# zaiisao/ConTEXTure-NeRF

Measured on AMD Instinct MI355X. Metric: UNet denoise steps/sec (CFG-batched SD2-depth UNet eval + PLMS update), higher is better.
Workload: dtype f16; 1 GPU; BASELINE configs[1]: 1 view @768^2 (latent 96^2), 50 PLMS steps (51 UNet evals), SD2-depth UNet fp16, CFG batch 2, guidance 10, random-init weights; mesh substitution napoleon.obj -> n/a for this stage (denoise loop only); latent=96, cfg_batch=2, ctx_len=77, views_per_rank=1, parallelism=view-shard x1

## Files before the change

contexture-nerf_amd/_lib.py:

```python
import ctypes as C
import os
import torch

_HERE = os.path.dirname(os.path.abspath(__file__))
LIB_PATH = os.path.join(_HERE, "libctxnerf.so")

_vp, _i32, _i64, _f32 = C.c_void_p, C.c_int32, C.c_int64, C.c_float

SIGNATURES = {
    "ctx_version": (_i32, []),
    "ctx_last_error": (C.c_char_p, []),
    "ctx_device_check": (_i32, []),
    "ctx_prepare_vertices": (_i32, [_vp, _vp, _vp, _vp, _i32, _i32, _i32, _vp, _vp, _vp, _vp, _vp]),
    "ctx_rasterize_ws_bytes": (_i64, [_i32, _i32, _i32, _i32]),
    "ctx_rasterize_fwd": (_i32, [_i32, _i32, _vp, _vp, _vp, _i32, _i32, _i32, _f32, _f32, _vp, _vp, _vp, _i64, _vp]),
    "ctx_rasterize_fused": (_i32, [_i32, _i32, _vp, _vp, _vp, _i32, _vp, _i32, _i32, _f32, _f32, _vp, _vp, _vp, _vp, _vp, _i64, _vp]),
    "ctx_normalize_depth_ws_bytes": (_i64, [_i32]),
    "ctx_normalize_depth": (_i32, [_vp, _i32, _i32, _vp, _vp, _vp, _vp]),
    "ctx_texture_mapping_fwd": (_i32, [_vp, _vp, _i32, _i32, _i32, _i32, _i32, _i32, _vp, _vp, _vp]),
    "ctx_texture_mapping_bwd": (_i32, [_vp, _vp, _i32, _i32, _i32, _i32, _vp, _vp, _vp]),
    "ctx_texmap_bwd_plan_bytes": (_i64, [_i32, _i32, _i32]),
    "ctx_texmap_bwd_plan": (_i32, [_vp, _vp, _i32, _i32, _i32, _vp, _vp]),
    "ctx_texture_mapping_bwd_binned_ws_bytes": (_i64, [_i32, _i32]),
    "ctx_texture_mapping_bwd_binned": (_i32, [_vp, _vp, _vp, _i32, _i32, _i32, _i32, _vp, _vp, _vp, _vp]),
# ... 86 lines not shown
    "ctx_unet_set_param": (_i32, [_vp, _i32, _vp, _vp]),
    "ctx_unet_forward": (_i32, [_vp, _vp, _vp, _vp, _i32, _i32, _i32, _i32, _vp, _vp]),
    "ctx_controlnet_create": (_vp, [_vp, _i32]),
    "ctx_controlnet_residual_bytes": (_i64, [_vp, _i32, _i32, _i32]),
    "ctx_controlnet_cond_cache_bytes": (_i64, [_vp, _i32, _i32, _i32]),
    "ctx_controlnet_forward": (_i32, [_vp, _vp, _vp, _vp, _vp, _vp, _i32, _i32, _i32, _i32, _i32, _vp, _vp]),
    "ctx_unet_set_residuals": (_i32, [_vp, _vp, C.c_float]),
    "ctx_unet_ref_bank_bytes": (_i64, [_vp, _i32, _i32, _i32]),
    "ctx_unet_workspace_bytes_ref": (_i64, [_vp, _i32, _i32, _i32, _i32, _i32, _i32]),
    "ctx_unet_forward_ref": (_i32, [_vp, _vp, _vp, _vp, _i32, _i32, _i32, _i32, _i32, _vp, _i32, _vp, _vp]),
    "ctx_unet_set_residual_fp32": (_i32, [_vp, _i32]),
    "ctx_unet_stats": (_i32, [_vp, _i32, _vp, _vp]),
    "ctx_unet_gn_epilogue_counts": (_i32, [_vp, _vp, _vp]),
    "ctx_unet_set_taps": (_i32, [_vp, _vp, _i64]),
    "ctx_unet_tap_count": (_i32, [_vp]),
    "ctx_unet_tap_info": (_i32, [_vp, _i32, _vp, _vp, _vp]),
    "ctx_vae_create": (_vp, [_vp]),
    "ctx_vae_destroy": (None, [_vp]),
    "ctx_vae_param_count": (_i32, [_vp]),
    "ctx_vae_param_name": (C.c_char_p, [_vp, _i32]),
    "ctx_vae_param_shape": (_i32, [_vp, _i32, _vp]),
    "ctx_vae_weight_bytes": (_i64, [_vp]),
    "ctx_vae_workspace_bytes": (_i64, [_vp, _i32, _i32, _i32]),
    "ctx_vae_bind": (_i32, [_vp, _vp, _vp, _i64]),
    "ctx_vae_derived_bytes": (_i64, [_vp]),
    "ctx_vae_bind_derived": (_i32, [_vp, _vp, _i64]),
    "ctx_vae_set_param": (_i32, [_vp, _i32, _vp, _vp]),
    "ctx_vae_decode": (_i32, [_vp, _vp, _i32, _i32, _i32, _vp, _vp]),
    "ctx_vae_decoder_param_count": (_i32, [_vp]),
    "ctx_vae_encode_workspace_bytes": (_i64, [_vp, _i32, _i32, _i32]),
    "ctx_vae_encode": (_i32, [_vp, _vp, _i32, _i32, _i32, _vp, _vp]),
    "ctx_vae_flops": (C.c_double, [_vp]),
    "ctx_vae_encode_train_workspace_bytes": (_i64, [_vp, _i32, _i32, _i32]),
    "ctx_vae_encode_train": (_i32, [_vp, _vp, _i32, _i32, _i32, _vp, _vp]),
    "ctx_vae_encode_bwd": (_i32, [_vp, _vp, _f32, _vp, _vp]),
    "ctx_gemm_f16": (_i32, [_vp, _vp, _vp, _vp, _i32, _i32, _i32, _vp, _vp]),
    "ctx_conv3x3_f16": (_i32, [_vp, _vp, _vp, _vp, _vp, _i32, _i32, _i32, _i32, _i32, _i32, _i32, _vp, _vp]),
    "ctx_conv3x3_seg_f16": (_i32, [_vp, _vp, _vp, _vp, _vp, _vp, _i32, _i32, _i32, _i32, _i32, _vp, _vp, _i32, _i32, _vp, _vp, _i32, _i32,
                                   _vp, _i32, _vp, _vp]),
    "ctx_conv3x3_gn_f16": (_i32, [_vp, _vp, _vp, _vp, _vp, _vp, _i32, _i32, _i32, _i32, _i32, _vp, _i32, _i32, _i32, _vp, _vp, _vp, _vp]),
    "ctx_gemm_last_kernel": (None, [_vp, _vp]),
    "ctx_conv3x3_geom_f16": (_i32, [_vp, _vp, _vp, _vp, _i32, _i32, _i32, _i32, _i32, _i32, _i32, _i32, _i32, _vp, _i32, _vp, _vp]),
    "ctx_pack_conv3_dgrad_f16": (_i32, [_vp, _i32, _i32, _i32, _vp, _vp]),
    "ctx_pack_conv3_phase_f16": (_i32, [_vp, _i32, _i32, _vp, _vp]),
    "ctx_conv3x3_phase_f16": (_i32, [_vp, _vp, _vp, _vp, _vp, _i32, _i32, _i32, _i32, _i32, _vp, _i32, _vp, _vp]),
    "ctx_pack_mat_dgrad_f16": (_i32, [_vp, _i32, _i32, _i32, _i32, _vp, _vp]),
    "ctx_groupnorm_bwd_ws_bytes": (_i64, [_i32, _i32]),
    "ctx_groupnorm_bwd_f16": (_i32, [_vp, _vp, _vp, _vp, _vp, _i32, _i32, _i32, _i32, _f32, _i32, _vp, _vp, _vp]),
    "ctx_softmax_rows_f16": (_i32, [_vp, _i32, _i32, _f32, _vp, _vp]),
    "ctx_softmax_bwd_rows_f16": (_i32, [_vp, _vp, _i32, _i32, _f32, _vp, _vp]),
    "ctx_quant_bwd_f16": (_i32, [_vp, _vp, _i32, _i32, _i64, _f32, _vp, _vp]),
    "ctx_conv_in_bwd_f16": (_i32, [_vp, _vp, _i32, _i32, _i32, _i32, _i32, _f32, _vp, _vp]),
    "ctx_conv_in_f16": (_i32, [_vp, _vp, _vp, _i32, _i32, _i32, _i32, _i32, _vp, _vp]),
    "ctx_conv_out_f16": (_i32, [_vp, _vp, _vp, _i32, _i32, _i32, _i32, _i32, _vp, _vp]),
    "ctx_gemv_f16": (_i32, [_vp, _vp, _vp, _i32, _i32, _i32, _i32, _i32, _vp, _vp]),
    "ctx_time_embed_f16": (_i32, [_vp, _i32, _i32, _vp, _vp]),
    "ctx_transpose_v_f16": (_i32, [_vp, _i32, _i32, _i32, _i32, _i32, _vp, _vp]),
    "ctx_concat_f16": (_i32, [_vp, _vp, _i64, _i32, _i32, _vp, _vp]),
    "ctx_concat_f32": (_i32, [_vp, _vp, _i64, _i32, _i32, _vp, _vp]),
    "ctx_f32_to_f16": (_i32, [_vp, _i64, _vp, _vp]),
    "ctx_f16_to_f32": (_i32, [_vp, _i64, _vp, _vp]),
    "ctx_conv_small_f16": (_i32, [_vp, _vp, _vp, _vp, _i32, _i32, _i32, _i32, _i32, _i32, _i32, _vp, _vp]),
    "ctx_add_scaled_f16": (_i32, [_vp, _vp, _f32, _i64, _vp]),
    "ctx_pointwise_f32": (_i32, [_vp, _vp, _vp, _i32, _i32, _i64, _i32, _vp, _vp]),
    "ctx_pack_fwd_f16": (_i32, [_vp, _i32, _i32, _i32, _vp, _vp]),
    "ctx_groupnorm_f16": (_i32, [_vp, _vp, _vp, _i32, _i32, _i32, _i32, _f32, _i32, _vp, _vp, _vp]),
    "ctx_groupnorm2_f16": (_i32, [_vp, _vp, _i32, _vp, _vp, _i32, _i32, _i32, _i32, _f32, _i32, _vp, _vp, _vp]),
    "ctx_groupnorm_apply_f16": (_i32, [_vp, _vp, _i32, _vp, _vp, _i32, _i32, _i32, _i32, _f32, _i32, _vp, _vp]),
    "ctx_groupnorm_slabs_f16": (_i32, [_vp, _i32, _vp, _vp, _vp, _i32, _vp, _vp, _i32, _i32, _i32, _i32, _f32, _i32, _vp, _vp]),
    "ctx_layernorm_f16": (_i32, [_vp, _vp, _vp, _i64, _i32, _f32, _vp, _vp]),
    "ctx_groupnorm_plan": (_i32, [_i32, _i32, _i32, _i32, _i32, _i32, _vp]),
    "ctx_layernorm_plan": (_i32, [_i64, _i32, _i32, _vp]),
    "ctx_groupnorm_f32in_f16": (_i32, [_vp, _vp, _vp, _i32, _i32, _i32, _i32, _f32, _i32, _vp, _vp, _vp]),
    "ctx_layernorm_f32in_f16": (_i32, [_vp, _vp, _vp, _i64, _i32, _f32, _vp, _vp]),
    "ctx_attention_ws_bytes": (_i64, [_i32, _i32, _i32]),
    "ctx_attention_f16": (_i32, [_vp, _vp, _vp, _i32, _i32, _i32, _i32, _i32, _i32, _f32, _vp, _i32, _vp, _vp]),
    "ctx_groupnorm_ws_bytes": (_i64, [_i32, _i32]),
    "ctx_geglu_f16": (_i32, [_vp, _i64, _i32, _vp, _vp]),
    "ctx_profile_begin": (_i32, []),
    "ctx_profile_end": (_i32, [_i32, _vp, _vp]),
    "ctx_bench_gemm": (C.c_float, [_vp, _vp, _vp, _vp, _i32, _i32, _i32, _vp, _i32, _i32, _i32, _i32, _i32, _i32, _vp, _i32, _i32, _vp]),
    "ctx_gemm_tune": (None, [_i32, _i32]),
    "ctx_attention_tune": (None, [_i32, _i32, _i32, _f32]),
    "ctx_probe_mfma": (_i32, [_i32, _vp, _vp, _vp, _vp]),
    "ctx_probe_stage": (C.c_float, [_i32, _i32, _i32, _i32, _i32, _vp, _vp, _vp]),
    "ctx_cfg_plms_step": (_i32, [_vp, _i64, _f32, _vp, _i32, _vp, _f32, _f32, _i32, _vp, _vp, _vp]),
}


class CtxError(RuntimeError):
    pass


_lib = None


def load():
    global _lib
    if _lib is None:
        if not os.path.exists(LIB_PATH):
            raise CtxError(f"{LIB_PATH} is missing: run `python -c 'import __graft_entry__ as g; g.build()'` "
                           "(hipcc --offload-arch=gfx950). There is no CPU fallback for this path.")
        lib = C.CDLL(LIB_PATH)
        for name, (res, args) in SIGNATURES.items():
            if not hasattr(lib, name) and os.environ.get("CTX_ALLOW_PARTIAL") == "1":
                continue
            fn = getattr(lib, name)
            fn.restype = res
            fn.argtypes = args
        _lib = lib
    return _lib


def check(rc):
    if rc != 0:
        raise CtxError(f"libctxnerf error {rc}: {load().ctx_last_error().decode()}")


def stream():
    return C.c_void_p(torch.cuda.current_stream().cuda_stream)


def ptr(t, dtype=None, name="tensor"):
    if t is None:
        return C.c_void_p(0)
    if not isinstance(t, torch.Tensor) or not t.is_cuda:
        raise CtxError(f"{name}: expected a device tensor (the HIP path has no CPU fallback), got "
                       f"{type(t).__name__} on {getattr(t, 'device', '?')}")
    if not t.is_contiguous():
        raise CtxError(f"{name}: tensor must be contiguous")
    if dtype is not None and t.dtype != dtype:
        raise CtxError(f"{name}: expected dtype {dtype}, got {t.dtype}")
    return C.c_void_p(t.data_ptr())


def f32c(t, device=None):
    t = t.to(dtype=torch.float32)
    if device is not None:
        t = t.to(device)
    return t.contiguous()
```

contexture-nerf_amd/csrc/attention.hip:

```cpp
#include "gemm_common.h"
#include <math.h>

#define AT_KB 64
#define AT_KROW 72
#define AT_VROW 68


struct AttnArgs {
    const f16 *Q, *K, *V;
    f16 *O;
    int Sq, Skv, heads;
    int q_stride, kv_stride, o_stride;
    float scale_log2e;
    float lazy;
};



typedef short at_s16x4 __attribute__((__vector_size__(4 * sizeof(short))));
__device__ __forceinline__ f16x4 at_tr16(const f16 *p)
{
    at_s16x4 v = __builtin_amdgcn_ds_read_tr16_b64_v4i16((__attribute__((address_space(3))) at_s16x4 *)p);
    return __builtin_bit_cast(f16x4, v);
}
struct AtNoIssue { __device__ __forceinline__ void operator()(int) const {} };
template <bool MASK, int NISSUE = 0, class Issue = AtNoIssue>
__device__ __forceinline__ void attn_tile(const f16 *__restrict__ Ks, const f16 *__restrict__ Vs, int k0, int Skv, int r, int h,
                                          int swz, int vlane, int vfq, float c, const f16x8 (&qf)[4], f32x16 (&o)[2], f32x16 &ls,
                                          float &m_run, float lazy, Issue iss = Issue())
{
    f32x16 s[2];
#pragma unroll
    for (int kb = 0; kb < 2; ++kb) {
#pragma unroll
        for (int q = 0; q < 16; ++q) s[kb][q] = 0.f;
        const f16 *kr = Ks + (kb * 32 + r) * 64;
#pragma unroll
        for (int ks = 0; ks < 4; ++ks) {
            f16x8 kf = *(const f16x8 *)(kr + ((2 * ks + h) ^ swz) * 8);
            s[kb] = __builtin_amdgcn_mfma_f32_32x32x16_f16(kf, qf[ks], s[kb], 0, 0, 0);
            if (kb * 4 + ks < NISSUE) iss(kb * 4 + ks);
        }
    }
    if (MASK) {
#pragma unroll
        for (int kb = 0; kb < 2; ++kb)
#pragma unroll
            for (int q = 0; q < 16; ++q) {
                int key = k0 + kb * 32 + (q & 3) + 8 * (q >> 2) + 4 * h;
                if (key >= Skv) s[kb][q] = -INFINITY;
            }
    }
    float mxa = fmaxf(s[0][0], s[0][1]), mxb = fmaxf(s[1][0], s[1][1]);
#pragma unroll
    for (int q = 2; q < 16; q += 2) {
        mxa = __builtin_fmaxf(__builtin_fmaxf(mxa, s[0][q]), s[0][q + 1]);
        mxb = __builtin_fmaxf(__builtin_fmaxf(mxb, s[1][q]), s[1][q + 1]);
    }
    float mx = fmaxf(mxa, mxb);
    mx = fmaxf(mx, __shfl_xor(mx, 32, 64)) * c;
    const float m_cand = fmaxf(m_run, mx);
    const bool move = __any(m_cand > m_run + lazy);
    const float m_new = move ? m_cand : m_run;
    typedef float at_f2 __attribute__((ext_vector_type(2)));
    const at_f2 c2 = {c, c}, nm2 = {-m_new, -m_new};
#pragma unroll
    for (int kb = 0; kb < 2; ++kb)
#pragma unroll
        for (int q = 0; q < 16; q += 2) {
            const at_f2 t = __builtin_elementwise_fma((at_f2){s[kb][q], s[kb][q + 1]}, c2, nm2);
            s[kb][q] = __builtin_amdgcn_exp2f(t[0]);
            s[kb][q + 1] = __builtin_amdgcn_exp2f(t[1]);
        }
    if (move) {
        const float alpha = __builtin_amdgcn_exp2f(m_run - m_new);
        asm volatile("s_nop 1\n\tv_mul_f32 %0, %0, %1" : "+v"(ls[0]) : "v"(alpha));
#pragma unroll
        for (int d = 0; d < 2; ++d)
#pragma unroll
            for (int q = 0; q < 16; ++q) asm volatile("v_mul_f32 %0, %0, %1" : "+v"(o[d][q]) : "v"(alpha));
    }
    m_run = m_new;
    const f16x8 ones = {1, 1, 1, 1, 1, 1, 1, 1};
#pragma unroll
    for (int kb = 0; kb < 2; ++kb)
#pragma unroll
        for (int st = 0; st < 2; ++st) {
            f16x8 pf;
#pragma unroll
            for (int j = 0; j < 8; ++j) pf[j] = (f16)s[kb][8 * st + j];
            const f16 *vk = Vs + (32 * kb + 16 * st + 4 * h) * 64 + vlane;
#pragma unroll
            for (int d = 0; d < 2; ++d) {
                const int co = ((4 * d) ^ vfq) * 8;
                f16x4 v0 = at_tr16(vk + co), v1 = at_tr16(vk + 8 * 64 + co);
                f16x8 vf = __builtin_shufflevector(v0, v1, 0, 1, 2, 3, 4, 5, 6, 7);
                o[d] = __builtin_amdgcn_mfma_f32_32x32x16_f16(vf, pf, o[d], 0, 0, 0);
            }
            ls = __builtin_amdgcn_mfma_f32_32x32x16_f16(ones, pf, ls, 0, 0, 0);
        }
}

template <int AT_NS, int NW, bool SPREAD = true>
__global__ __launch_bounds__(64 * NW, NW == 8 ? 4 : 1) void k_attention_dma(AttnArgs a)
{
    __shared__ __attribute__((aligned(16))) f16 ring[AT_NS * 2 * 64 * 64];
    const int tid = threadIdx.x, lane = tid & 63, wave = __builtin_amdgcn_readfirstlane(tid >> 6);
    const int r = lane & 31, h = lane >> 5;
    const int b = blockIdx.z, hd = blockIdx.y;
    const int q0 = blockIdx.x * (32 * NW) + wave * 32;
    const int qrow = q0 + r;
    const bool qok = qrow < a.Sq;
    constexpr int PI = 8 / NW;
    constexpr int G = 2 * PI;

    f16x8 qf[4];
    const f16x8 zero8 = {0, 0, 0, 0, 0, 0, 0, 0};
    {
        const f16 *qp = a.Q + ((size_t)b * a.Sq + (qok ? qrow : 0)) * a.q_stride + hd * 64 + 8 * h;
#pragma unroll
        for (int ks = 0; ks < 4; ++ks) qf[ks] = qok ? *(const f16x8 *)(qp + ks * 16) : zero8;
    }
    f32x16 o[2];
#pragma unroll
    for (int d = 0; d < 2; ++d)
#pragma unroll
        for (int q = 0; q < 16; ++q) o[d][q] = 0.f;
    f32x16 ls;
#pragma unroll
    for (int q = 0; q < 16; ++q) ls[q] = 0.f;
    float m_run = -INFINITY;

    const int ntiles = (a.Skv + AT_KB - 1) / AT_KB;
    const int lr = lane >> 3, pc = lane & 7;
    const f16 *kp[PI], *vp[PI];
    int krow[PI];
#pragma unroll
    for (int i = 0; i < PI; ++i) {
        int row = 8 * (wave + NW * i) + lr;
        int lc = (pc ^ ((row >> 1) & 7)) * 8;
        krow[i] = row;
        kp[i] = a.K + ((size_t)b * a.Skv + row) * a.kv_stride + hd * 64 + lc;
        vp[i] = a.V + ((size_t)b * a.Skv + row) * a.kv_stride + hd * 64 + ((pc ^ (((row >> 1) & 1) << 2)) * 8);
    }
    int issued = 0;
    auto issue = [&](int buf) {
        f16 *Ks = ring + buf * (2 * 64 * 64);
        f16 *Vs = Ks + 64 * 64;
        const int k0 = issued * AT_KB;
#pragma unroll
        for (int i = 0; i < PI; ++i) {
            const f16 *src = (k0 + krow[i] < a.Skv) ? kp[i] : ctx_zero_page;
            __builtin_amdgcn_global_load_lds((gptr_t)src, (lptr_t)(Ks + (wave + NW * i) * 512), 16, 0, 0);
            kp[i] += (size_t)AT_KB * a.kv_stride;
        }
#pragma unroll
        for (int i = 0; i < PI; ++i) {
            const f16 *src = (k0 + krow[i] < a.Skv) ? vp[i] : ctx_zero_page;
            __builtin_amdgcn_global_load_lds((gptr_t)src, (lptr_t)(Vs + (wave + NW * i) * 512), 16, 0, 0);
            vp[i] += (size_t)AT_KB * a.kv_stride;
        }
        ++issued;
    };
    auto issue_piece = [&](int buf, int idx) {
        f16 *Ks = ring + buf * (2 * 64 * 64);
        f16 *Vs = Ks + 64 * 64;
        const int k0 = issued * AT_KB;
        const int i = idx < PI ? idx : idx - PI;
        const f16 *&gp = idx < PI ? kp[i] : vp[i];
        const f16 *src = (k0 + krow[i] < a.Skv) ? gp : ctx_zero_page;
        __builtin_amdgcn_global_load_lds((gptr_t)src, (lptr_t)((idx < PI ? Ks : Vs) + (wave + NW * i) * 512), 16, 0, 0);
        gp += (size_t)AT_KB * a.kv_stride;
    };
#pragma unroll
    for (int p = 0; p < AT_NS - 1; ++p)
        if (p < ntiles) issue(p);

    const int swz = (r >> 1) & 7;
    const int vq = (lane & 15) >> 2, vfq = ((vq >> 1) & 1) << 2;
    const int vlane = vq * 64 + (((2 * ((lane >> 4) & 1) + ((lane & 3) >> 1)) ^ 0) * 8) + (lane & 1) * 4;
    const float c = a.scale_log2e;
    const int nfull = a.Skv / AT_KB;
    int slot = 0;
    int t = 0;
    for (; t < nfull && t + AT_NS - 1 < ntiles; ++t) {
        asm volatile("s_waitcnt vmcnt(%0)" ::"n"((AT_NS - 2) * G) : "memory");
        __builtin_amdgcn_sched_barrier(0);
        ctx_barrier();
        const int ibuf = slot == 0 ? AT_NS - 1 : slot - 1;
        const f16 *Ks = ring + slot * (2 * 64 * 64);
        if (SPREAD) {
            attn_tile<false, G>(Ks, Ks + 64 * 64, t * AT_KB, a.Skv, r, h, swz, vlane, vfq, c, qf, o, ls, m_run, a.lazy, [&](int idx) { issue_piece(ibuf, idx); });
            ++issued;
        } else {
            issue(ibuf);
            attn_tile<false>(Ks, Ks + 64 * 64, t * AT_KB, a.Skv, r, h, swz, vlane, vfq, c, qf, o, ls, m_run, a.lazy);
        }
        slot = slot + 1 == AT_NS ? 0 : slot + 1;
    }
    for (; t < nfull; ++t) {
        const int newer = issued - 1 - t;
        if (AT_NS >= 4 && newer >= 2) asm volatile("s_waitcnt vmcnt(%0)" ::"n"(2 * G) : "memory");
        else if (newer >= 1) asm volatile("s_waitcnt vmcnt(%0)" ::"n"(G) : "memory");
        else asm volatile("s_waitcnt vmcnt(0)" ::: "memory");
        __builtin_amdgcn_sched_barrier(0);
        ctx_barrier();
        if (issued < ntiles) issue(slot == 0 ? AT_NS - 1 : slot - 1);
        const f16 *Ks = ring + slot * (2 * 64 * 64);
        attn_tile<false>(Ks, Ks + 64 * 64, t * AT_KB, a.Skv, r, h, swz, vlane, vfq, c, qf, o, ls, m_run, a.lazy);
        slot = slot + 1 == AT_NS ? 0 : slot + 1;
    }
    if (nfull < ntiles) {
        asm volatile("s_waitcnt vmcnt(0)" ::: "memory");
        ctx_barrier();
        const f16 *Ks = ring + slot * (2 * 64 * 64);
        attn_tile<true>(Ks, Ks + 64 * 64, nfull * AT_KB, a.Skv, r, h, swz, vlane, vfq, c, qf, o, ls, m_run, a.lazy);
    }
    if (qok) {
        float inv = 1.0f / ls[0];
        f16 *op = a.O + ((size_t)b * a.Sq + qrow) * a.o_stride + hd * 64;
#pragma unroll
        for (int d = 0; d < 2; ++d)
#pragma unroll
            for (int g = 0; g < 4; ++g) {
                f16x4 v;
#pragma unroll
                for (int j = 0; j < 4; ++j) v[j] = (f16)(o[d][4 * g + j] * inv);
                *(f16x4 *)(op + d * 32 + 8 * g + 4 * h) = v;
            }
    }
}

template <int NS, int NW, bool SPREAD = true>
static void attn_launch(const AttnArgs &a, int B, bool report, hipStream_t s)
{
    constexpr auto kern = k_attention_dma<NS, NW, SPREAD>;
    if (report) {
        int nb = 0;
        hipFuncAttributes fa;
        (void)hipOccupancyMaxActiveBlocksPerMultiprocessor(&nb, kern, 64 * NW, 0);
        (void)hipFuncGetAttributes(&fa, (const void *)kern);
        fprintf(stderr, "[ctx] attention: %d blocks/CU by the occupancy API, %d VGPRs, %zu B static LDS\n", nb, fa.numRegs, fa.sharedSizeBytes);
    }
    ctx_launch<kern>(1, dim3(cdiv(a.Sq, 32 * NW), a.heads, B), dim3(64 * NW), 0, s, a);
}

struct AttnTune { int ns, nw8, spread; float lazy; };
static AttnTune g_attn_force = {-1, -1, -1, -1.f};
static const AttnTune &attn_tune_env()
{
    static const AttnTune env = [] {
        AttnTune t;
        t.ns = ctx_env_int("CTX_ATTN_NS", 3);
        t.nw8 = ctx_env_int("CTX_ATTN_NW8", -1);
        t.spread = ctx_env_int("CTX_ATTN_SPREAD", 1);
        const char *e = getenv("CTX_ATTN_LAZY");
        t.lazy = e ? (float)atof(e) : 8.0f;
        if (!(t.lazy >= 0.f && t.lazy <= 12.f)) t.lazy = 8.0f;
        return t;
    }();
    return env;
}

extern "C" void ctx_attention_tune(int32_t ns, int32_t nw8, int32_t spread, float lazy)
{
    g_attn_force.ns = ns; g_attn_force.nw8 = nw8; g_attn_force.spread = spread; g_attn_force.lazy = lazy;
}

int ctx_attention_core(const f16 *Q, const f16 *K, const f16 *V, int B, int Sq, int Skv, int heads, int q_stride,
                       int kv_stride, float scale, f16 *O, int o_stride, hipStream_t s)
{
    AttnArgs a;
    a.Q = Q; a.K = K; a.V = V; a.O = O; a.Sq = Sq; a.Skv = Skv; a.heads = heads;
    a.q_stride = q_stride; a.kv_stride = kv_stride; a.o_stride = o_stride;
    a.scale_log2e = scale * 1.4426950408889634f;
    const AttnTune &tu = attn_tune_env();
    const float lazy = g_attn_force.lazy >= 0.f ? g_attn_force.lazy : tu.lazy;
    a.lazy = lazy >= 0.f && lazy <= 12.f ? lazy : 8.0f;
    const int ns = g_attn_force.ns >= 0 ? g_attn_force.ns : tu.ns;
    const int nw8 = g_attn_force.nw8 >= 0 ? g_attn_force.nw8 : tu.nw8;
    const bool w8 = nw8 == 1 || (nw8 < 0 && Sq >= 1024 && Sq < 4096 && Skv >= 1024);
    const int spread = g_attn_force.spread >= 0 ? g_attn_force.spread : tu.spread;
    static int dbg = -1;
    bool report = false;
    if (dbg < 0) { dbg = ctx_env_int("CTX_ATTN_DEBUG", 0); report = dbg != 0; }
    if (w8) {
        if (ns == 2) attn_launch<2, 8>(a, B, report, s); else if (ns == 4) attn_launch<4, 8>(a, B, report, s);
        else if (spread) attn_launch<3, 8>(a, B, report, s); else attn_launch<3, 8, false>(a, B, report, s);
    } else {
        if (ns == 2) attn_launch<2, 4>(a, B, report, s); else if (ns == 4) attn_launch<4, 4>(a, B, report, s);
        else if (spread) attn_launch<3, 4>(a, B, report, s); else attn_launch<3, 4, false>(a, B, report, s);
    }
    hipError_t e = hipGetLastError();
    if (e != hipSuccess) {
        ctx_set_error("attention launch failed: %s", hipGetErrorString(e));
        return CTX_E_LAUNCH;
    }
    return CTX_OK;
}

extern "C" int64_t ctx_attention_ws_bytes(int32_t B, int32_t Skv, int32_t heads)
{
    (void)B; (void)Skv; (void)heads;
    return 256;
}

extern "C" int32_t ctx_attention_f16(const void *Q, const void *K, const void *V, int32_t B, int32_t Sq, int32_t Skv,
                                     int32_t heads, int32_t q_stride, int32_t kv_stride, float scale, void *O,
                                     int32_t o_stride, void *vt_ws, ctx_stream_t stream)
{
    (void)vt_ws;
    CTX_REQUIRE(Q && K && V && O, "attention: null pointer");
    CTX_REQUIRE(B > 0 && Sq > 0 && Skv > 0 && heads > 0 && q_stride % 8 == 0 && kv_stride % 8 == 0 && o_stride % 4 == 0 &&
                    q_stride >= heads * 64 && kv_stride >= heads * 64 && o_stride >= heads * 64,
                "attention: bad strides/sizes (head_dim is fixed at 64)");
    return ctx_attention_core((const f16 *)Q, (const f16 *)K, (const f16 *)V, B, Sq, Skv, heads, q_stride, kv_stride, scale, (f16 *)O,
                              o_stride, (hipStream_t)stream);
}
```

include/ctx_nerf.h:

```cpp
#ifndef CTX_NERF_H
#define CTX_NERF_H
#include <stdint.h>
#ifdef __cplusplus
extern "C" {
#endif

#define CTX_OK 0
#define CTX_E_ARG (-1)
#define CTX_E_LAUNCH (-2)
#define CTX_E_STATE (-3)

typedef void *ctx_stream_t;

int32_t ctx_version(void);
const char *ctx_last_error(void);
int32_t ctx_device_check(void);

int32_t ctx_prepare_vertices(const float *verts, const int64_t *faces, const float *cam,
                             const float *proj3, int32_t B, int32_t V, int32_t F,
                             float *fv_cam, float *fv_img, float *fnorm,
                             void *ws , ctx_stream_t stream);

int64_t ctx_rasterize_ws_bytes(int32_t H, int32_t W, int32_t B, int32_t F);
int32_t ctx_rasterize_fwd(int32_t H, int32_t W, const float *face_z, const float *face_xy,
// ... 277 lines not shown
int32_t ctx_conv3x3_seg_f16(const void *x, const void *w, const void *bias, const void *bias2, const void *rowbias,
                            const void *residual, int32_t B, int32_t H, int32_t W, int32_t Cin, int32_t Cout,
                            const void *xa, const void *wa, int32_t Ca, int32_t ldwa, const void *xb, const void *wb,
                            int32_t Cb, int32_t ldwb, void *part, int32_t splitk, void *y, ctx_stream_t stream);
int32_t ctx_conv3x3_gn_f16(const void *x, const void *w, const void *bias, const void *bias2, const void *rowbias,
                           const void *residual, int32_t B, int32_t H, int32_t W, int32_t Cin, int32_t Cout, void *part,
                           int32_t splitk, int32_t keep_slabs, int32_t groups, void *gn_part, int32_t *slots, void *y,
                           ctx_stream_t stream);
void ctx_gemm_last_kernel(int32_t *tile, int32_t *use8);
int32_t ctx_conv3x3_geom_f16(const void *x, const void *w, const void *bias, const void *residual, int32_t B, int32_t H, int32_t W,
                             int32_t Cin, int32_t Cout, int32_t stride, int32_t upsample, int32_t poff, int32_t zins, void *part,
                             int32_t splitk, void *y, ctx_stream_t stream);
int32_t ctx_pack_conv3_phase_f16(const float *src, int32_t Cout, int32_t Cin, void *dst, ctx_stream_t stream);
int32_t ctx_conv3x3_phase_f16(const void *x, const void *wp, const void *bias, const void *rowbias, const void *residual, int32_t B,
                              int32_t H, int32_t W, int32_t Cin, int32_t Cout, void *part, int32_t splitk, void *y, ctx_stream_t stream);
int32_t ctx_pack_conv3_dgrad_f16(const float *src, int32_t Cout, int32_t Cin, int32_t pad, void *dst, ctx_stream_t stream);
int32_t ctx_pack_mat_dgrad_f16(const float *src, int32_t out, int32_t in, int32_t ld, int32_t col, void *dst, ctx_stream_t stream);
int64_t ctx_groupnorm_bwd_ws_bytes(int32_t B, int32_t groups);
int32_t ctx_groupnorm_bwd_f16(const void *x, const void *dy, const void *gamma, const void *beta, const void *add, int32_t B, int32_t HW,
                              int32_t C, int32_t groups, float eps, int32_t silu, void *dx, void *ws, ctx_stream_t stream);
int32_t ctx_softmax_rows_f16(const void *s, int32_t rows, int32_t n, float scale, void *p, ctx_stream_t stream);
int32_t ctx_softmax_bwd_rows_f16(const void *P, const void *dP, int32_t rows, int32_t n, float scale, void *dS, ctx_stream_t stream);
int32_t ctx_quant_bwd_f16(const float *g, const void *w, int32_t B, int32_t C, int64_t HW, float gscale, void *d, ctx_stream_t stream);
int32_t ctx_conv_in_bwd_f16(const void *dy, const void *w_pack, int32_t B, int32_t H, int32_t W, int32_t C, int32_t Cimg, float inv_gscale,
                            float *dimg, ctx_stream_t stream);
int32_t ctx_conv_in_f16(const float *x, const void *w_pack, const void *bias, int32_t B, int32_t Cin, int32_t H, int32_t W, int32_t Cout,
                        void *y, ctx_stream_t stream);
int32_t ctx_conv_out_f16(const void *x, const void *w, const void *bias, int32_t B, int32_t H, int32_t W, int32_t C, int32_t Cout,
                         float *out, ctx_stream_t stream);
int32_t ctx_gemv_f16(const void *x, const void *w, const void *bias, int32_t Bm, int32_t N, int32_t K, int32_t silu_in, int32_t silu_out,
                     void *out, ctx_stream_t stream);
int32_t ctx_time_embed_f16(const float *t, int32_t B, int32_t dim, void *out, ctx_stream_t stream);
int32_t ctx_transpose_v_f16(const void *v, int32_t B, int32_t S, int32_t ld, int32_t heads, int32_t Sp, void *vt, ctx_stream_t stream);
int32_t ctx_concat_f16(const void *a, const void *b, int64_t M, int32_t Ca, int32_t Cb, void *y, ctx_stream_t stream);
int32_t ctx_concat_f32(const float *a, const float *b, int64_t M, int32_t Ca, int32_t Cb, float *y, ctx_stream_t stream);
int32_t ctx_f32_to_f16(const float *x, int64_t n, void *y, ctx_stream_t stream);
int32_t ctx_f16_to_f32(const void *x, int64_t n, float *y, ctx_stream_t stream);
int32_t ctx_conv_small_f16(const float *x32, const void *x16, const void *w, const void *bias, int32_t B, int32_t H, int32_t W, int32_t Cin,
                           int32_t Cout, int32_t stride, int32_t silu, void *y, ctx_stream_t stream);
int32_t ctx_add_scaled_f16(void *dst, const void *src, float scale, int64_t n, ctx_stream_t stream);
int32_t ctx_pointwise_f32(const void *x, const void *w, const void *b, int32_t B, int32_t C, int64_t HW, int32_t nhwc16, float *y,
                          ctx_stream_t stream);
int32_t ctx_pack_fwd_f16(const float *src, int32_t kind, int32_t a, int32_t b, void *dst, ctx_stream_t stream);
int64_t ctx_groupnorm_ws_bytes(int32_t B, int32_t groups);
int32_t ctx_groupnorm_f16(const void *x, const void *gamma, const void *beta, int32_t B, int32_t HW,
                          int32_t C, int32_t groups, float eps, int32_t silu, void *y, void *stats_ws,
                          ctx_stream_t stream);
int32_t ctx_groupnorm2_f16(const void *xa, const void *xb, int32_t Ca, const void *gamma, const void *beta, int32_t B,
                           int32_t HW, int32_t C, int32_t groups, float eps, int32_t silu, void *y, void *stats_ws,
                           ctx_stream_t stream);
int32_t ctx_groupnorm_apply_f16(const void *x, const void *part, int32_t slots, const void *gamma, const void *beta, int32_t B,
                                int32_t HW, int32_t C, int32_t groups, float eps, int32_t silu, void *y, ctx_stream_t stream);
int32_t ctx_groupnorm_slabs_f16(const void *part, int32_t splitk, const void *bias, const void *bias2, const void *rowbias,
                                int32_t ldrb, const void *gamma, const void *beta, int32_t B, int32_t HW, int32_t C,
                                int32_t groups, float eps, int32_t silu, void *y, ctx_stream_t stream);
int32_t ctx_layernorm_f16(const void *x, const void *gamma, const void *beta, int64_t rows, int32_t C,
                          float eps, void *y, ctx_stream_t stream);
int32_t ctx_groupnorm_plan(int32_t B, int32_t HW, int32_t C, int32_t groups, int32_t x32, int32_t Ca, int32_t *out);
int32_t ctx_layernorm_plan(int64_t rows, int32_t C, int32_t x32, int64_t *out);
int32_t ctx_groupnorm_f32in_f16(const float *x, const void *gamma, const void *beta, int32_t B, int32_t HW, int32_t C,
                                int32_t groups, float eps, int32_t silu, void *y, void *stats_ws, ctx_stream_t stream);
int32_t ctx_layernorm_f32in_f16(const float *x, const void *gamma, const void *beta, int64_t rows, int32_t C, float eps,
                                void *y, ctx_stream_t stream);
int64_t ctx_attention_ws_bytes(int32_t B, int32_t Skv, int32_t heads);
int32_t ctx_attention_f16(const void *Q, const void *K, const void *V, int32_t B, int32_t Sq, int32_t Skv,
                          int32_t heads, int32_t q_stride, int32_t kv_stride, float scale, void *O,
                          int32_t o_stride, void *vt_ws, ctx_stream_t stream);
int32_t ctx_geglu_f16(const void *h, int64_t M, int32_t C4, void *y, ctx_stream_t stream);

int32_t ctx_cfg_plms_step(const float *eps_pair, int64_t n, float guidance, float *ets, int32_t head,
                          const float *coef4, float sample_coeff, float eps_coeff, int32_t mode,
                          float *cur_sample_ws, float *x, ctx_stream_t stream);

int32_t ctx_profile_begin(void);
int32_t ctx_profile_end(int32_t klass, double *total_ms , int64_t *count );

float ctx_bench_gemm(const void *A, const void *Wt, const void *bias, const void *residual, int32_t M, int32_t N, int32_t K,
                     void *C, int32_t conv_B, int32_t conv_H, int32_t conv_W, int32_t conv_Cin, int32_t conv_flags, int32_t epi,
                     void *part, int32_t splitk, int32_t iters, ctx_stream_t stream);

void ctx_gemm_tune(int32_t tile, int32_t gemm8);

void ctx_attention_tune(int32_t ns, int32_t nw8, int32_t spread, float lazy);

int32_t ctx_probe_mfma(int32_t which, const void *A, const void *Bt, float *C, ctx_stream_t stream);

float ctx_probe_stage(int32_t mode, int32_t waves, int32_t u, int32_t iters, int32_t shared_region, const void *src, void *sink,
                      ctx_stream_t stream);

#ifdef __cplusplus
}
#endif
#endif
```

Measured before the change: 121.7 steps/s.

## Add split-KV 12-wave attention variant with cost-model launch planner

Adds a KV-split attention kernel shape: 12 waves per workgroup, with two halves each streaming half of the KV tiles into their own LDS rings. The halves then merge their softmax partials (o, l, m) through LDS. A cost model chooses between 4-wave, 8-wave and split 12-wave launches from workgroup count versus CU count, to fill the GPU better on small-Sq, long-Skv shapes. The DMA addressing is reworked into SGPR base plus VGPR offset pieces, and the cross-half max shuffle is swapped for ds_bpermute. The cost is more LDS, a merge step and extra barriers.

```diff
diff --git a/contexture-nerf_amd/_lib.py b/contexture-nerf_amd/_lib.py
--- a/contexture-nerf_amd/_lib.py
+++ b/contexture-nerf_amd/_lib.py
@@ -192,6 +192,7 @@
     "ctx_bench_gemm": (C.c_float, [_vp, _vp, _vp, _vp, _i32, _i32, _i32, _vp, _i32, _i32, _i32, _i32, _i32, _i32, _vp, _i32, _i32, _vp]),
     "ctx_gemm_tune": (None, [_i32, _i32]),
     "ctx_attention_tune": (None, [_i32, _i32, _i32, _f32]),
+    "ctx_attention_plan": (_i32, [_i32, _i32, _i32, _i32, _i32, _vp]),
     "ctx_probe_mfma": (_i32, [_i32, _vp, _vp, _vp, _vp]),
     "ctx_probe_stage": (C.c_float, [_i32, _i32, _i32, _i32, _i32, _vp, _vp, _vp]),
     "ctx_cfg_plms_step": (_i32, [_vp, _i64, _f32, _vp, _i32, _vp, _f32, _f32, _i32, _vp, _vp, _vp]),
diff --git a/contexture-nerf_amd/csrc/attention.hip b/contexture-nerf_amd/csrc/attention.hip
--- a/contexture-nerf_amd/csrc/attention.hip
+++ b/contexture-nerf_amd/csrc/attention.hip
@@ -1,5 +1,6 @@
 #include "gemm_common.h"
 #include <math.h>
+#include <type_traits>
 
 #define AT_KB 64
 #define AT_KROW 72
@@ -26,7 +27,7 @@
 struct AtNoIssue { __device__ __forceinline__ void operator()(int) const {} };
 template <bool MASK, int NISSUE = 0, class Issue = AtNoIssue>
 __device__ __forceinline__ void attn_tile(const f16 *__restrict__ Ks, const f16 *__restrict__ Vs, int k0, int Skv, int r, int h,
-                                          int swz, int vlane, int vfq, float c, const f16x8 (&qf)[4], f32x16 (&o)[2], f32x16 &ls,
+                                          int swz, int vlane, int vfq, int xidx, float c, const f16x8 (&qf)[4], f32x16 (&o)[2], f32x16 &ls,
                                           float &m_run, float lazy, Issue iss = Issue())
 {
     f32x16 s[2];
@@ -58,7 +59,7 @@
         mxb = __builtin_fmaxf(__builtin_fmaxf(mxb, s[1][q]), s[1][q + 1]);
     }
     float mx = fmaxf(mxa, mxb);
-    mx = fmaxf(mx, __shfl_xor(mx, 32, 64)) * c;
+    mx = fmaxf(mx, __builtin_bit_cast(float, __builtin_amdgcn_ds_bpermute(xidx, __builtin_bit_cast(int, mx)))) * c;
     const float m_cand = fmaxf(m_run, mx);
     const bool move = __any(m_cand > m_run + lazy);
     const float m_new = move ? m_cand : m_run;
@@ -101,18 +102,21 @@
         }
 }
 
-template <int AT_NS, int NW, bool SPREAD = true>
-__global__ __launch_bounds__(64 * NW, NW == 8 ? 4 : 1) void k_attention_dma(AttnArgs a)
-{
-    __shared__ __attribute__((aligned(16))) f16 ring[AT_NS * 2 * 64 * 64];
+template <int AT_NS, int NW, bool SPREAD = true, int KS = 1>
+__global__ __launch_bounds__(64 * NW, NW == 8 ? 4 : NW == 12 ? 3 : 1) void k_attention_dma(AttnArgs a)
+{
+    constexpr int NQ = NW / KS;
+    constexpr int STAGE = 2 * 64 * 64;
+    constexpr int G = (16 + NQ - 1) / NQ;
+    static_assert(NW == NQ * KS && (KS == 1 ? 16 % NQ == 0 : NQ * 34 * 64 * 4 <= KS * 2 * STAGE * 2), "attention: workgroup shape");
+    __shared__ __attribute__((aligned(16))) f16 ring[KS * AT_NS * STAGE];
     const int tid = threadIdx.x, lane = tid & 63, wave = __builtin_amdgcn_readfirstlane(tid >> 6);
+    const int half = KS == 1 ? 0 : (wave >= NQ ? 1 : 0), qw = wave - half * NQ;
     const int r = lane & 31, h = lane >> 5;
     const int b = blockIdx.z, hd = blockIdx.y;
-    const int q0 = blockIdx.x * (32 * NW) + wave * 32;
+    const int q0 = blockIdx.x * (32 * NQ) + qw * 32;
     const int qrow = q0 + r;
     const bool qok = qrow < a.Sq;
-    constexpr int PI = 8 / NW;
-    constexpr int G = 2 * PI;
 
     f16x8 qf[4];
     const f16x8 zero8 = {0, 0, 0, 0, 0, 0, 0, 0};
@@ -132,89 +136,109 @@
     float m_run = -INFINITY;
 
     const int ntiles = (a.Skv + AT_KB - 1) / AT_KB;
+    const int nmax = (ntiles + KS - 1) / KS;
+    const int tb = half * nmax, n = half ? ntiles - nmax : nmax;
+    const int nf = max(min(tb + n, a.Skv / AT_KB) - tb, 0);
+    f16 *const ringh = ring + half * (AT_NS * STAGE);
     const int lr = lane >> 3, pc = lane & 7;
-    const f16 *kp[PI], *vp[PI];
-    int krow[PI];
-#pragma unroll
-    for (int i = 0; i < PI; ++i) {
-        int row = 8 * (wave + NW * i) + lr;
-        int lc = (pc ^ ((row >> 1) & 7)) * 8;
-        krow[i] = row;
-        kp[i] = a.K + ((size_t)b * a.Skv + row) * a.kv_stride + hd * 64 + lc;
-        vp[i] = a.V + ((size_t)b * a.Skv + row) * a.kv_stride + hd * 64 + ((pc ^ (((row >> 1) & 1) << 2)) * 8);
-    }
+    const char *dsrc[G];
+    uint32_t doff[G];
+    int drow[G], dlds[G];
+#pragma unroll
+    for (int j = 0; j < G; ++j) {
+        const int p = (KS > 1 && qw + NQ * j >= 16) ? qw : qw + NQ * j;
+        const bool isv = KS == 1 ? j >= G / 2 : p >= 8;
+        const int row = 8 * (p & 7) + lr;
+        const int lc = isv ? pc ^ (((row >> 1) & 1) << 2) : pc ^ ((row >> 1) & 7);
+        drow[j] = row;
+        doff[j] = ((uint32_t)row * (uint32_t)a.kv_stride + lc * 8) * 2;
+        dlds[j] = (isv ? 64 * 64 : 0) + (p & 7) * 512;
+        dsrc[j] = (const char *)((isv ? a.V : a.K) + ((size_t)b * a.Skv + (size_t)tb * AT_KB) * a.kv_stride + hd * 64);
+    }
+    const size_t tile_bytes = (size_t)AT_KB * a.kv_stride * 2;
     int issued = 0;
-    auto issue = [&](int buf) {
-        f16 *Ks = ring + buf * (2 * 64 * 64);
-        f16 *Vs = Ks + 64 * 64;
-        const int k0 = issued * AT_KB;
-#pragma unroll
-        for (int i = 0; i < PI; ++i) {
-            const f16 *src = (k0 + krow[i] < a.Skv) ? kp[i] : ctx_zero_page;
-            __builtin_amdgcn_global_load_lds((gptr_t)src, (lptr_t)(Ks + (wave + NW * i) * 512), 16, 0, 0);
-            kp[i] += (size_t)AT_KB * a.kv_stride;
-        }
-#pragma unroll
-        for (int i = 0; i < PI; ++i) {
-            const f16 *src = (k0 + krow[i] < a.Skv) ? vp[i] : ctx_zero_page;
-            __builtin_amdgcn_global_load_lds((gptr_t)src, (lptr_t)(Vs + (wave + NW * i) * 512), 16, 0, 0);
-            vp[i] += (size_t)AT_KB * a.kv_stride;
-        }
+    auto issue_piece = [&](int buf, int j, auto full) {
+        asm volatile("" : "+s"(dsrc[j]), "+v"(doff[j]));
+        const char *src = dsrc[j] + (size_t)doff[j];
+        if (!decltype(full)::value && (tb + issued) * AT_KB + drow[j] >= a.Skv) src = (const char *)ctx_zero_page;
+        __builtin_amdgcn_global_load_lds((gptr_t)src, (lptr_t)(ringh + buf * STAGE + dlds[j]), 16, 0, 0);
+        dsrc[j] += tile_bytes;
+    };
+    auto issue = [&](int buf, auto full) {
+#pragma unroll
+        for (int j = 0; j < G; ++j) issue_piece(buf, j, full);
         ++issued;
     };
-    auto issue_piece = [&](int buf, int idx) {
-        f16 *Ks = ring + buf * (2 * 64 * 64);
-        f16 *Vs = Ks + 64 * 64;
-        const int k0 = issued * AT_KB;
-        const int i = idx < PI ? idx : idx - PI;
-        const f16 *&gp = idx < PI ? kp[i] : vp[i];
-        const f16 *src = (k0 + krow[i] < a.Skv) ? gp : ctx_zero_page;
-        __builtin_amdgcn_global_load_lds((gptr_t)src, (lptr_t)((idx < PI ? Ks : Vs) + (wave + NW * i) * 512), 16, 0, 0);
-        gp += (size_t)AT_KB * a.kv_stride;
-    };
+    constexpr std::true_type FULL{};
+    constexpr std::false_type ANY{};
 #pragma unroll
     for (int p = 0; p < AT_NS - 1; ++p)
-        if (p < ntiles) issue(p);
+        if (p < n) issue(p, ANY);
 
     const int swz = (r >> 1) & 7;
     const int vq = (lane & 15) >> 2, vfq = ((vq >> 1) & 1) << 2;
     const int vlane = vq * 64 + (((2 * ((lane >> 4) & 1) + ((lane & 3) >> 1)) ^ 0) * 8) + (lane & 1) * 4;
+    const int xidx = (lane ^ 32) << 2;
     const float c = a.scale_log2e;
-    const int nfull = a.Skv / AT_KB;
     int slot = 0;
     int t = 0;
-    for (; t < nfull && t + AT_NS - 1 < ntiles; ++t) {
+    for (; t + AT_NS - 1 < nf; ++t) {
         asm volatile("s_waitcnt vmcnt(%0)" ::"n"((AT_NS - 2) * G) : "memory");
         __builtin_amdgcn_sched_barrier(0);
         ctx_barrier();
         const int ibuf = slot == 0 ? AT_NS - 1 : slot - 1;
-        const f16 *Ks = ring + slot * (2 * 64 * 64);
+        const f16 *Ks = ringh + slot * STAGE;
         if (SPREAD) {
-            attn_tile<false, G>(Ks, Ks + 64 * 64, t * AT_KB, a.Skv, r, h, swz, vlane, vfq, c, qf, o, ls, m_run, a.lazy, [&](int idx) { issue_piece(ibuf, idx); });
+            attn_tile<false, G>(Ks, Ks + 64 * 64, (tb + t) * AT_KB, a.Skv, r, h, swz, vlane, vfq, xidx, c, qf, o, ls, m_run, a.lazy,
+                                [&](int idx) { issue_piece(ibuf, idx, FULL); });
             ++issued;
         } else {
-            issue(ibuf);
-            attn_tile<false>(Ks, Ks + 64 * 64, t * AT_KB, a.Skv, r, h, swz, vlane, vfq, c, qf, o, ls, m_run, a.lazy);
+            issue(ibuf, FULL);
+            attn_tile<false>(Ks, Ks + 64 * 64, (tb + t) * AT_KB, a.Skv, r, h, swz, vlane, vfq, xidx, c, qf, o, ls, m_run, a.lazy);
         }
         slot = slot + 1 == AT_NS ? 0 : slot + 1;
     }
-    for (; t < nfull; ++t) {
+    for (; t < nf; ++t) {
         const int newer = issued - 1 - t;
         if (AT_NS >= 4 && newer >= 2) asm volatile("s_waitcnt vmcnt(%0)" ::"n"(2 * G) : "memory");
         else if (newer >= 1) asm volatile("s_waitcnt vmcnt(%0)" ::"n"(G) : "memory");
         else asm volatile("s_waitcnt vmcnt(0)" ::: "memory");
         __builtin_amdgcn_sched_barrier(0);
         ctx_barrier();
-        if (issued < ntiles) issue(slot == 0 ? AT_NS - 1 : slot - 1);
-        const f16 *Ks = ring + slot * (2 * 64 * 64);
-        attn_tile<false>(Ks, Ks + 64 * 64, t * AT_KB, a.Skv, r, h, swz, vlane, vfq, c, qf, o, ls, m_run, a.lazy);
+        if (issued < n) issue(slot == 0 ? AT_NS - 1 : slot - 1, ANY);
+        const f16 *Ks = ringh + slot * STAGE;
+        attn_tile<false>(Ks, Ks + 64 * 64, (tb + t) * AT_KB, a.Skv, r, h, swz, vlane, vfq, xidx, c, qf, o, ls, m_run, a.lazy);
         slot = slot + 1 == AT_NS ? 0 : slot + 1;
     }
-    if (nfull < ntiles) {
+    if (nf < n) {
         asm volatile("s_waitcnt vmcnt(0)" ::: "memory");
         ctx_barrier();
-        const f16 *Ks = ring + slot * (2 * 64 * 64);
-        attn_tile<true>(Ks, Ks + 64 * 64, nfull * AT_KB, a.Skv, r, h, swz, vlane, vfq, c, qf, o, ls, m_run, a.lazy);
+        const f16 *Ks = ringh + slot * STAGE;
+        attn_tile<true>(Ks, Ks + 64 * 64, (tb + nf) * AT_KB, a.Skv, r, h, swz, vlane, vfq, xidx, c, qf, o, ls, m_run, a.lazy);
+    }
+    if (KS > 1) {
+        for (int i = n; i < nmax; ++i) ctx_barrier();
+        float *mg = (float *)ring + qw * (34 * 64) + lane;
+        asm volatile("s_waitcnt lgkmcnt(0)" ::: "memory");
+        ctx_barrier();
+        if (half) {
+#pragma unroll
+            for (int d = 0; d < 2; ++d)
+#pragma unroll
+                for (int q = 0; q < 16; ++q) mg[(16 * d + q) * 64] = o[d][q];
+            mg[32 * 64] = ls[0];
+            mg[33 * 64] = m_run;
+        }
+        asm volatile("s_waitcnt lgkmcnt(0)" ::: "memory");
+        ctx_barrier();
+        if (half) return;
+        const float m1 = mg[33 * 64], m = fmaxf(m_run, m1);
+        const float a0 = __builtin_amdgcn_exp2f(m_run - m), a1 = m1 == -INFINITY ? 0.f : __builtin_amdgcn_exp2f(m1 - m);
+        ls[0] = ls[0] * a0 + mg[32 * 64] * a1;
+#pragma unroll
+        for (int d = 0; d < 2; ++d)
+#pragma unroll
+            for (int q = 0; q < 16; ++q) o[d][q] = o[d][q] * a0 + mg[(16 * d + q) * 64] * a1;
     }
     if (qok) {
         float inv = 1.0f / ls[0];
@@ -231,10 +255,10 @@
     }
 }
 
-template <int NS, int NW, bool SPREAD = true>
+template <int NS, int NW, bool SPREAD = true, int KS = 1>
 static void attn_launch(const AttnArgs &a, int B, bool report, hipStream_t s)
 {
-    constexpr auto kern = k_attention_dma<NS, NW, SPREAD>;
+    constexpr auto kern = k_attention_dma<NS, NW, SPREAD, KS>;
     if (report) {
         int nb = 0;
         hipFuncAttributes fa;
@@ -242,7 +266,36 @@
         (void)hipFuncGetAttributes(&fa, (const void *)kern);
         fprintf(stderr, "[ctx] attention: %d blocks/CU by the occupancy API, %d VGPRs, %zu B static LDS\n", nb, fa.numRegs, fa.sharedSizeBytes);
     }
-    ctx_launch<kern>(1, dim3(cdiv(a.Sq, 32 * NW), a.heads, B), dim3(64 * NW), 0, s, a);
+    ctx_launch<kern>(1, dim3(cdiv(a.Sq, 32 * NW / KS), a.heads, B), dim3(64 * NW), 0, s, a);
+}
+
+struct AttnPlan { int nw, ks, wgs, cost; };
+static AttnPlan attn_plan(int B, int Sq, int Skv, int heads, int n_cu, int nw8)
+{
+    const int ntiles = cdiv(Skv, AT_KB);
+    auto form = [&](int nw, int ks) {
+        AttnPlan p = {nw, ks, cdiv(Sq, 32 * nw / ks) * heads * B, 0};
+        const int64_t cost = (int64_t)cdiv(p.wgs, n_cu) * (nw / 4) * (cdiv(ntiles, ks) + (ks > 1 ? 1 : 0));
+        p.cost = (int)(cost < INT32_MAX ? cost : INT32_MAX);
+        return p;
+    };
+    const AttnPlan f4 = form(4, 1), f8 = form(8, 1), f12 = form(12, 2);
+    if (nw8 >= 0) return nw8 == 2 ? f12 : nw8 == 1 ? f8 : f4;
+    const bool w8 = Sq >= 1024 && Sq < 4096 && Skv >= 1024;
+    AttnPlan best = w8 ? f8 : f4;
+    const int64_t bar = (int64_t)best.cost * 7;
+    for (const AttnPlan &p : {f4, f8, f12})
+        if ((int64_t)p.cost * 8 < bar && p.cost < best.cost) best = p;
+    return best;
+}
+static int attn_cu_count()
+{
+    static const int n = [] {
+        int dev = 0, cu = 0;
+        if (hipGetDevice(&dev) != hipSuccess || hipDeviceGetAttribute(&cu, hipDeviceAttributeMultiprocessorCount, dev) != hipSuccess || cu <= 0) cu = 256;
+        return cu;
+    }();
+    return n;
 }
 
 struct AttnTune { int ns, nw8, spread; float lazy; };
@@ -266,6 +319,15 @@
 {
     g_attn_force.ns = ns; g_attn_force.nw8 = nw8; g_attn_force.spread = spread; g_attn_force.lazy = lazy;
 }
+static int attn_nw8() { return g_attn_force.nw8 >= 0 ? g_attn_force.nw8 : attn_tune_env().nw8; }
+
+extern "C" int32_t ctx_attention_plan(int32_t B, int32_t Sq, int32_t Skv, int32_t heads, int32_t n_cu, int32_t *out)
+{
+    CTX_REQUIRE(out && B > 0 && Sq > 0 && Skv > 0 && heads > 0 && n_cu > 0, "attention plan: bad arguments");
+    const AttnPlan p = attn_plan(B, Sq, Skv, heads, n_cu, attn_nw8());
+    out[0] = p.nw; out[1] = p.ks; out[2] = p.wgs; out[3] = p.cost;
+    return CTX_OK;
+}
 
 int ctx_attention_core(const f16 *Q, const f16 *K, const f16 *V, int B, int Sq, int Skv, int heads, int q_stride,
                        int kv_stride, float scale, f16 *O, int o_stride, hipStream_t s)
@@ -278,13 +340,15 @@
     const float lazy = g_attn_force.lazy >= 0.f ? g_attn_force.lazy : tu.lazy;
     a.lazy = lazy >= 0.f && lazy <= 12.f ? lazy : 8.0f;
     const int ns = g_attn_force.ns >= 0 ? g_attn_force.ns : tu.ns;
-    const int nw8 = g_attn_force.nw8 >= 0 ? g_attn_force.nw8 : tu.nw8;
-    const bool w8 = nw8 == 1 || (nw8 < 0 && Sq >= 1024 && Sq < 4096 && Skv >= 1024);
+    const AttnPlan plan = attn_plan(B, Sq, Skv, heads, attn_cu_count(), attn_nw8());
     const int spread = g_attn_force.spread >= 0 ? g_attn_force.spread : tu.spread;
     static int dbg = -1;
     bool report = false;
     if (dbg < 0) { dbg = ctx_env_int("CTX_ATTN_DEBUG", 0); report = dbg != 0; }
-    if (w8) {
+    if (plan.ks == 2) {
+        if (ns == 2) attn_launch<2, 12, true, 2>(a, B, report, s); else if (ns == 4) attn_launch<4, 12, true, 2>(a, B, report, s);
+        else if (spread) attn_launch<3, 12, true, 2>(a, B, report, s); else attn_launch<3, 12, false, 2>(a, B, report, s);
+    } else if (plan.nw == 8) {
         if (ns == 2) attn_launch<2, 8>(a, B, report, s); else if (ns == 4) attn_launch<4, 8>(a, B, report, s);
         else if (spread) attn_launch<3, 8>(a, B, report, s); else attn_launch<3, 8, false>(a, B, report, s);
     } else {
@@ -314,6 +378,7 @@
     CTX_REQUIRE(B > 0 && Sq > 0 && Skv > 0 && heads > 0 && q_stride % 8 == 0 && kv_stride % 8 == 0 && o_stride % 4 == 0 &&
                     q_stride >= heads * 64 && kv_stride >= heads * 64 && o_stride >= heads * 64,
                 "attention: bad strides/sizes (head_dim is fixed at 64)");
+    CTX_REQUIRE(kv_stride < (1 << 24), "attention: kv_stride %d is beyond the 2^24 elements the tile addressing holds", kv_stride);
     return ctx_attention_core((const f16 *)Q, (const f16 *)K, (const f16 *)V, B, Sq, Skv, heads, q_stride, kv_stride, scale, (f16 *)O,
                               o_stride, (hipStream_t)stream);
 }
diff --git a/include/ctx_nerf.h b/include/ctx_nerf.h
--- a/include/ctx_nerf.h
+++ b/include/ctx_nerf.h
@@ -383,6 +383,7 @@
 void ctx_gemm_tune(int32_t tile, int32_t gemm8);
 
 void ctx_attention_tune(int32_t ns, int32_t nw8, int32_t spread, float lazy);
+int32_t ctx_attention_plan(int32_t B, int32_t Sq, int32_t Skv, int32_t heads, int32_t n_cu, int32_t *out);
 
 int32_t ctx_probe_mfma(int32_t which, const void *A, const void *Bt, float *C, ctx_stream_t stream);
 
```

New measurement: 123.6 steps/s, median of 6. 1.5% higher.
